# mkofler96/DeepSDF

Hardware: AMD Instinct MI355X
Metric: SDF point-samples/sec per training step (8x512 decoder, 16384 pts) (higher is better)
Workload: dtype f32; 1 GPU; configs[1]: 64 synthetic sphere-SDF scenes, latent_dim=256, 8x512 decoder + layer-4 skip, weight-norm, dropout 0.2, 16384 pts/step (64 scenes x 256 samples), fp32; headline_config=True, parallelism=dp1

## Files before the change

deepsdf_amd/csrc/dsdf_api.hip:

```cpp
#include "../../include/dsdf.h"

#include <hip/hip_runtime.h>
#include <math.h>
#include <stdarg.h>
#include <stdio.h>
#include <string.h>

#include <stdlib.h>

#include <algorithm>
#include <atomic>

#include "dwstream.hpp"
#include "sample.hpp"
#include "fused.hpp"
#include "fused_bf16x8.hpp"
#include "gemm.hpp"
#include "kernels.hpp"
#include "mcubes.hpp"
#include "meshsdf.hpp"
#include "msgrid.hpp"

using namespace dsdf;

// ... 240 lines not shown
}

std::atomic<size_t> g_redzone{0};
struct WsRow { const char* name; int idx; size_t off, bytes; };
struct WsTable {
  int n, dropped;
  size_t total;
  WsRow row[DSDF_WS_MAX_REGIONS];
  void reset() { n = 0; dropped = 0; total = 0; }
  void add(const char* name, int idx, size_t off, size_t bytes) {
    if (n < DSDF_WS_MAX_REGIONS) row[n++] = WsRow{name, idx, off, bytes};
    else ++dropped;
  }
};
thread_local WsTable t_last_plan;

struct Plan {
  int nl, W0, N, R;
  int ld_in[DSDF_MAX_LAYERS];
  size_t in_off[DSDF_MAX_LAYERS];
  int ld_dp, ldz, ldcs, ld_part, last_blocks, nsplit, kchunk, mt;
  long long slab;
  size_t u_off, y_off, dp_off[2], dzA_off, dzB_off, slab_off, colsum_off, part_off, part2_off, partdb_off,
      partloss_off, segpart_off, segnorm_off, gnorm_off, dxz_off[2], lnpg_off, lnpb_off, total;
  size_t lnx_off[DSDF_MAX_LAYERS], lnr_off[DSDF_MAX_LAYERS];
  size_t dpl_off[DSDF_MAX_LAYERS], mask_off[DSDF_MAX_LAYERS], cs_off[DSDF_MAX_LAYERS], dwslab_off[DSDF_MAX_LAYERS];
  int nwg, frows;
  DwSched dw;
  DwSched dwph[DSDF_MAX_BUCKETS];
  int dw_nb, dw_cut[DSDF_MAX_BUCKETS + 1];
  int segmode, ldu, ldh;
  long long hstride;
  size_t hoistU_off, xsum_off[2], hs_off, zr_off;
};

Plan make_plan(const DsdfNet* n, int64_t N, int64_t R, bool inference, bool segmode = false, int nb = 2, int frows = FROWS,
               WsTable* rec = nullptr) {
  Plan P;
  memset(&P, 0, sizeof(P));
  P.frows = frows;
  P.nl = n->n_layers; P.W0 = n->latent_size + n->geom_dim; P.N = (int)N; P.R = (int)R;
  size_t o = 0;
  const size_t guard = g_redzone.load(std::memory_order_relaxed);
  if (rec) rec->reset();
  auto take = [&](const char* name, int idx, size_t bytes) {
    size_t r = o;
    o += (size_t)rup((int64_t)bytes, 256) + guard;
    if (rec) rec->add(name, idx, r, bytes);
    return r;
  };
  int maxw = 4;
  for (int l = 0; l < P.nl; ++l) {
    P.ld_in[l] = (int)rup(n->in_dim[l], 4);
    if (P.ld_in[l] > maxw) maxw = P.ld_in[l];
  }
  if (inference) {
// ... 33 lines not shown
  int maxout = 1;
  for (int l = 0; l < P.nl - 1; ++l) {
    const int64_t s = (int64_t)n->out_dim[l] * P.ld_in[l];
    if (s > maxslab) maxslab = s;
    if (n->out_dim[l] > maxout) maxout = n->out_dim[l];
  }
  P.slab = rup(maxslab, 64);
  P.slab_off = take("slab", -1, (size_t)P.nsplit * P.slab * 4);
  P.mt = (int)((N + BM - 1) / BM);
  P.ldcs = (int)rup(maxout, 4);
  P.colsum_off = take("colsum", -1, (size_t)P.mt * P.ldcs * 4);
  if (n->ln_param_mask) { P.lnpg_off = take("lnpg", -1, (size_t)LN_BLOCKS * P.ldcs * 4); P.lnpb_off = take("lnpb", -1, (size_t)LN_BLOCKS * P.ldcs * 4); }
  P.last_blocks = (int)((N + 15) / 16);
  if (P.last_blocks > LAST_BLOCKS_MAX) P.last_blocks = LAST_BLOCKS_MAX;
  if (P.last_blocks < 1) P.last_blocks = 1;
  P.ld_part = 2 * P.ld_in[P.nl - 1];
  const size_t part_rows = (size_t)std::max<int64_t>(P.last_blocks, (N + frows - 1) / frows);
  P.part_off = take("part", -1, part_rows * P.ld_part * 4);
  P.part2_off = take("part2", -1, (size_t)LAST_GROUPS * P.ld_part * 4);
  P.partdb_off = take("partdb", -1, part_rows * 4);
  P.partloss_off = take("partloss", -1, part_rows * 4);
  P.segpart_off = take("segpart", -1, (size_t)LAT_SLICES_MAX * (R > 0 ? R : 1) * (n->latent_size > 0 ? n->latent_size : 1) * 4);
  P.segnorm_off = take("segnorm", -1, (size_t)(R > 0 ? R : 1) * 4);
  P.gnorm_off = take("gnorm", -1, 1024 * 4);
  P.nwg = (int)((N + frows - 1) / frows);
  for (int l = 0; l < P.nl - 1; ++l) {
    P.dpl_off[l] = take("dpl", l, (size_t)N * maxw * 4 + 4096);
    P.mask_off[l] = take("mask", l, (size_t)P.nwg * 256 * 16);
    P.cs_off[l] = take("cs", l, (size_t)P.nwg * P.ldcs * 4);
  }
  P.dw = dw_schedule(n, N, P.ld_in, segmode);
  P.dw_nb = nb < 2 ? 2 : (nb > DSDF_MAX_BUCKETS ? DSDF_MAX_BUCKETS : nb);
  dw_bucket_cuts(n, P.dw_nb, P.dw_cut);
  for (int t = 0; t < P.dw_nb; ++t)
    P.dwph[t] = dw_schedule(n, N, P.ld_in, segmode, P.dw_cut[t + 1], P.dw_cut[t],
                            t == 0 && P.dw_nb == 2 && segmode && P.nwg <= chip_waves() / 4 ? 64 : 0);
  for (int l = 0; l < P.nl - 1; ++l) {
    int ns = P.dw.nsplit[l];
    for (int t = 0; t < P.dw_nb; ++t)
      if (P.dwph[t].nsplit[l] > ns) ns = P.dwph[t].nsplit[l];
    P.dwslab_off[l] = take("dwslab", l, (size_t)ns * P.dw.slab[l] * 4);
  }
  P.segmode = segmode ? 1 : 0;
  if (segmode) {
    P.ldu = P.ldcs;
    P.hoistU_off = take("hoistU", -1, (size_t)(R > 0 ? R : 1) * 2 * P.ldu * 4);
    for (int t = 0; t < 2; ++t) P.xsum_off[t] = take("xsum", t, (size_t)P.nwg * 4 * P.ldcs * 4);
// ... 41 lines not shown
int launch_last(const LastArgs& a, int blocks, hipStream_t st) {
  if (a.n <= 0) return 0;
  const int in = a.in;
  ProfScope ps(DSDF_PROF_LAST, (MODE == LAST_FWD ? 2.0 : 6.0) * a.n * a.in, st);
  if (in <= 256) hipLaunchKernelGGL((last_layer_kernel<MODE, 1>), dim3(blocks), dim3(256), 0, st, a);
  else if (in <= 512) hipLaunchKernelGGL((last_layer_kernel<MODE, 2>), dim3(blocks), dim3(256), 0, st, a);
  else if (in <= 1024) hipLaunchKernelGGL((last_layer_kernel<MODE, 4>), dim3(blocks), dim3(256), 0, st, a);
  else hipLaunchKernelGGL((last_layer_kernel<MODE, 8>), dim3(blocks), dim3(256), 0, st, a);
  LAUNCH_OK("last_layer_kernel");
  return 0;
}

AdamRide adam_ride(float* p, const float* g, float* m, float* v, int64_t n, float lr, const DsdfAdamCfg* c) {
  AdamRide a;
  memset(&a, 0, sizeof(a));
  const double bc1 = 1.0 - pow((double)c->beta1, (double)c->step), bc2 = 1.0 - pow((double)c->beta2, (double)c->step);
  a.p = p; a.g = g; a.m = m; a.v = v; a.n = n;
  a.blocks = (int)((n + 255) / 256 < 2048 ? (n + 255) / 256 : 2048);
  a.omb1 = 1.0f - c->beta1; a.b2 = c->beta2; a.omb2 = 1.0f - c->beta2;
  a.step_size = (float)((double)lr / bc1); a.bc2_sqrt = (float)sqrt(bc2); a.eps = c->eps;
  return a;
}

int materialize(const DsdfNet* net, const float* params, float* packed, hipStream_t st, bool scales_ready = false,
                const AdamRide* ride = nullptr) {
  DsdfParamLayout L;
  param_layout(net, &L);
  const Packed pk = packed_layout(net);
  WnAll a;
  memset(&a, 0, sizeof(a));
  a.nl = net->n_layers;
  a.scale = packed + pk.scale_off;
  int rows = 0, tiles = 0;
  for (int l = 0; l < net->n_layers; ++l) {
    WnLayer& y = a.ly[l];
    y.v = params + L.v_off[l];
    y.g = L.g_off[l] >= 0 ? params + L.g_off[l] : nullptr;
    y.W = packed + pk.w_off[l];
    y.WT = (l == net->n_layers - 1) ? nullptr : packed + pk.wt_off[l];
    y.out = net->out_dim[l]; y.in = net->in_dim[l]; y.ldw = pk.ldw[l]; y.ldwt = pk.ldwt[l];
    y.row0 = rows; y.tile0 = tiles; y.tcols = (y.in + 31) / 32;
    const bool last = l == net->n_layers - 1;
    y.Wf = last ? nullptr : packed + pk.wf_off[l];
    y.WTf = last ? nullptr : packed + pk.wtf_off[l];
    y.Wfb = (last || !net->fwd_bf16) ? nullptr : reinterpret_cast<__bf16*>(packed + pk.wfb_off[l]);
    y.Uf = pk.uf[l]; y.UTf = pk.utf[l];
    const bool sp = net->gemm_split && !last;
    y.Ws = sp ? reinterpret_cast<__bf16*>(packed + pk.ws_off[l]) : nullptr;
    y.WTs = sp ? reinterpret_cast<__bf16*>(packed + pk.wts_off[l]) : nullptr;
    y.ws_plane = pk.ws_plane[l]; y.wts_plane = pk.wts_plane[l];
    rows += y.out;
    tiles += ((y.out + 31) / 32) * y.tcols;
  }
  a.total_rows = rows; a.total_tiles = tiles;
  if (!scales_ready) {
    hipLaunchKernelGGL(wn_scale_kernel, dim3((rows + 3) / 4), dim3(256), 0, st, a);
    LAUNCH_OK("wn_scale_kernel");
  }
  if (ride != nullptr) a.adam = *ride;
  hipLaunchKernelGGL(wn_tiles_kernel, dim3(tiles + a.adam.blocks), dim3(256), 0, st, a);
  LAUNCH_OK("wn_tiles_kernel");
  return 0;
}

constexpr float LATENT_DROPOUT_P = 0.2f;
constexpr int LATENT_DROPOUT_KEY = DSDF_MAX_LAYERS - 1;
inline uint32_t latent_drop_thr() { return (uint32_t)lround((double)LATENT_DROPOUT_P * 65536.0); }
inline bool net_variant(const DsdfNet* n) { return n->latent_dropout || n->xyz_in_all || n->ln_param_mask != 0; }
inline bool ln_applied(const DsdfNet* n, int l) { return ((n->ln_param_mask >> l) & 1) && l < n->n_layers - 1; }


int run_gather(const DsdfNet* net, const Plan& P, void* ws, const float* table, const DsdfBatch* b, const float* input,
               int64_t ld_in, int64_t n, hipStream_t st, int training = 0, const uint32_t* keys = nullptr, uint32_t row_offset = 0) {
  GatherArgs g;
  memset(&g, 0, sizeof(g));
  g.table = table; g.L = net->latent_size; g.G = net->geom_dim;
  if (b) { g.xyz = b->xyz; g.seg_scene = b->seg_scene; g.seg_offset = b->seg_offset; g.R = (int)b->n_segments; }
// ... 57 lines not shown
int run_hoist(const DsdfNet* net, const Plan& P, void* ws, const float* packed, const float* table, const DsdfBatch* b,
              FusedSeg* seg, hipStream_t st, const HoistRenorm* renorm = nullptr) {
  if (net->latent_size < 1 || net->latent_size > HOIST_MAXL)
    return fail(DSDF_E_INVALID, "segment mode needs 1 <= latent_size <= %d (got %d)", HOIST_MAXL, net->latent_size);
  const Packed pk = packed_layout(net);
  const int ks = skip_layer(net);
  HoistArgs h;
  memset(&h, 0, sizeof(h));
  memset(seg, 0, sizeof(*seg));
  h.nh = ks > 0 ? 2 : 1;
  h.W[0] = packed + pk.w_off[0]; h.ldw[0] = pk.ldw[0]; h.c0[0] = 0; h.out[0] = net->out_dim[0];
  seg->h[0].layer = 0; seg->h[0].wx = h.W[0] + net->latent_size; seg->h[0].ldw = pk.ldw[0];
  seg->h[1].layer = -1;
  if (ks > 0) {
    h.W[1] = packed + pk.w_off[ks]; h.ldw[1] = pk.ldw[ks]; h.c0[1] = net->out_dim[ks - 1]; h.out[1] = net->out_dim[ks];
    seg->h[1].layer = ks; seg->h[1].wx = h.W[1] + h.c0[1] + net->latent_size; seg->h[1].ldw = pk.ldw[ks];
  }
  h.L = net->latent_size; h.seg_scene = b->seg_scene; h.table = table; h.R = (int)b->n_segments;
  h.U = at<float>(ws, P.hoistU_off); h.ldu = P.ldu;
  h.bf16 = net->fwd_bf16 ? 1 : 0;
  if (renorm != nullptr) {
    h.max_norm = renorm->max_norm; h.zr = at<float>(ws, P.zr_off);
    h.dlat = renorm->nzero > 0 ? renorm->dlat : nullptr; h.nzero = renorm->nzero;
  }
  const int rows = h.out[0] + (ks > 0 ? h.out[1] : 0);
  const dim3 hgrid((unsigned)((rows + 3) / 4), (unsigned)((h.R + HOIST_SC - 1) / HOIST_SC));
  switch ((h.L + 63) >> 6) {
    case 1: hipLaunchKernelGGL(seg_hoist_kernel<1>, hgrid, dim3(256), 0, st, h); break;
    case 2: hipLaunchKernelGGL(seg_hoist_kernel<2>, hgrid, dim3(256), 0, st, h); break;
    case 3: case 4: hipLaunchKernelGGL(seg_hoist_kernel<4>, hgrid, dim3(256), 0, st, h); break;
    default: hipLaunchKernelGGL(seg_hoist_kernel<8>, hgrid, dim3(256), 0, st, h); break;
  }
  LAUNCH_OK("seg_hoist_kernel");
  seg->wg_per_seg = (int)(b->seg_len / P.frows);
  seg->xyz = b->xyz; seg->G = net->geom_dim; seg->U = h.U; seg->ldu = h.ldu;
  return 0;
}

int run_fused_forward(const DsdfNet* net, const Plan& P, void* ws, const float* packed, const float* params, int64_t n,
                      int training, const uint32_t* keys, uint32_t row_offset, bool store_act, float* y_out, float* u_out,
                      hipStream_t st, const FusedSeg* seg = nullptr, FusedFwdArgs* defer = nullptr) {
  DsdfParamLayout L;
  param_layout(net, &L);
  const Packed pk = packed_layout(net);
  const int last = net->n_layers - 1;
  FusedFwdArgs a;
// ... 214 lines not shown
      TRY(launch_nt<EPI_BWD>(a, st));
      if (want_xyz) {
        const long long tot = (long long)n * net->geom_dim;
        hipLaunchKernelGGL(acc_cols_kernel, dim3((unsigned)((tot + 255) / 256)), dim3(256), 0, st, at<float>(ws, P.dxz_off[0]), 4,
                           at<float>(ws, P.dxz_off[1]), 4, 0, (int)n, net->geom_dim, *xyz_acc ? 1 : 0);
        LAUNCH_OK("acc_cols_kernel");
        *xyz_acc = true;
      }
      cur ^= 1;
    } else if (ncols_dz > 0) {
      a.C = at<float>(ws, P.dzA_off); a.ldc = P.ldz; a.N = ncols_dz;
      TRY(launch_nt<EPI_PLAIN>(a, st));
      if (net->latent_dropout && training && keys != nullptr && net->latent_size > 0) {
        const long long tot = (long long)n * net->latent_size;
        hipLaunchKernelGGL(latent_drop_bwd_kernel, dim3((unsigned)((tot + 255) / 256)), dim3(256), 0, st, at<float>(ws, P.dzA_off), P.ldz,
                           (int)n, net->latent_size, keys[LATENT_DROPOUT_KEY], latent_drop_thr(), 1.0f / (1.0f - LATENT_DROPOUT_P), row_offset);
        LAUNCH_OK("latent_drop_bwd_kernel");
      }
    }
  }
  return 0;
}

struct FuseAdam { const DsdfAdamCfg* cfg; float* params; float* exp_avg; float* exp_avg_sq; float* packed; };

struct SegBwd { const FusedSeg* seg; const int64_t* seg_scene; const float* table; int R;
                ScatterArgs* scatter; bool* scatter_done;
                const float* zr; };

int run_backward_fused(const DsdfNet* net, const Plan& P, void* ws, const float* packed, const float* params, int64_t n,
                       int training, float* grads, int accumulate, int ncols_dz, bool* used_dzB, hipStream_t st,
                       bool want_dw, const FusedBwdHead& head, const FuseAdam* fz = nullptr, const SegBwd* sb = nullptr,
                       const FusedFwdArgs* fwd = nullptr,
                       int phase = 0) {
  const DwSched& DS = phase == 0 ? P.dw : P.dwph[phase - 1];
  auto in_phase = [&](int l) { return phase == 0 || (l >= P.dw_cut[phase] && l < P.dw_cut[phase - 1]); };
  DsdfParamLayout L;
  param_layout(net, &L);
  const Packed pk = packed_layout(net);
  const int nl = net->n_layers, last = nl - 1;
  *used_dzB = false;
  FusedBwdArgs a;
  memset(&a, 0, sizeof(a));
  a.N = (int)n;
  a.head = head;
  const bool segmode = sb != nullptr;
  const int ks = skip_layer(net);
// ... 192 lines not shown
      if (segmode && (l == 0 || l == ks)) {
        f.hoist = 1; f.lat0 = l == 0 ? 0 : net->out_dim[l - 1]; f.hW = net->latent_size + net->geom_dim; f.ldh = P.ldh;
        f.hs = at<float>(ws, P.hs_off) + (l == 0 ? 0 : P.hstride);
      }
      if (fz != nullptr) {
        const DsdfAdamCfg* c = fz->cfg;
        const double bc1 = 1.0 - pow((double)c->beta1, (double)c->step), bc2 = 1.0 - pow((double)c->beta2, (double)c->step);
        f.adam = 1;
        f.pb = fz->params + L.bias_off[l]; f.mb = fz->exp_avg + L.bias_off[l]; f.sb = fz->exp_avg_sq + L.bias_off[l];
        f.pv = fz->params + L.v_off[l];    f.mv = fz->exp_avg + L.v_off[l];    f.sv = fz->exp_avg_sq + L.v_off[l];
        if (L.g_off[l] >= 0) { f.pg = fz->params + L.g_off[l]; f.mg = fz->exp_avg + L.g_off[l]; f.sg = fz->exp_avg_sq + L.g_off[l]; }
        int r0 = 0;
        for (int q = 0; q < l; ++q) r0 += net->out_dim[q];
        f.scale_out = fz->packed + pk.scale_off + r0;
        f.omb1 = 1.0f - c->beta1; f.b2 = c->beta2; f.omb2 = 1.0f - c->beta2;
        f.step_size = (float)((double)c->lr_decoder / bc1); f.bc2_sqrt = (float)sqrt(bc2); f.eps = c->eps;
      }
      fa.row0[fa.n] = rows;
      rows += fin_blocks(f.out, f.in);
      ++fa.n;
    }
    fa.row0[fa.n] = rows;
    if (rows == 0) return 0;
    if (segmode && sb->scatter != nullptr && phase <= 1) {
      hipLaunchKernelGGL(finalize_scatter_kernel, dim3(rows + sb->R), dim3(256), 0, st, fa, *sb->scatter, rows);
      LAUNCH_OK("finalize_scatter_kernel");
      *sb->scatter_done = true;
    } else {
      hipLaunchKernelGGL(finalize_all_kernel, dim3(rows), dim3(256), 0, st, fa);
      LAUNCH_OK("finalize_all_kernel");
    }
  }
  return 0;
}

FusedBwdHead make_head(const DsdfNet* net, const Plan& P, void* ws, const float* packed, const float* params, int mode,
                       int training) {
  DsdfParamLayout L;
  param_layout(net, &L);
  const Packed pk = packed_layout(net);
  const int last = net->n_layers - 1;
  FusedBwdHead h;
  memset(&h, 0, sizeof(h));
  h.mode = mode;
  h.a_last = at<float>(ws, P.in_off[last]); h.ld_a = P.ld_in[last]; h.in_last = net->in_dim[last];
  h.w_last = packed + pk.w_off[last]; h.b_last = params + L.bias_off[last]; h.use_tanh = net->use_tanh;
  h.mask_scale = mask_scale_of(net, last - 1, training);
// ... 600 lines not shown
    }
    a.total_rows = rows;
    hipLaunchKernelGGL(adam_rows_kernel, dim3((rows + 3) / 4), dim3(256), 0, st, a);
    LAUNCH_OK("adam_rows_kernel");
    for (int l = 0; l < net->n_layers; ++l)
      if (L.ln_w_off[l] >= 0)
        TRY(adam_launch(params + L.ln_w_off[l], grads + L.ln_w_off[l], exp_avg + L.ln_w_off[l], exp_avg_sq + L.ln_w_off[l],
                        2 * (int64_t)net->out_dim[l], cfg->lr_decoder, cfg, cfg->grad_scale, st));
  }
  if (n_latent_floats > 0) {
    if (!latent_table || !dlat || !lat_exp_avg || !lat_exp_avg_sq) return fail(DSDF_E_INVALID, "NULL latent argument");
    const AdamRide ride = adam_ride(latent_table, dlat, lat_exp_avg, lat_exp_avg_sq, n_latent_floats, cfg->lr_latent, cfg);
    return materialize(net, params, packed, st, true, &ride);
  }
  return materialize(net, params, packed, st, true);
}

int dsdf_train_step(const DsdfNet* net, float* packed, float* params, float* grads, float* exp_avg, float* exp_avg_sq,
                    float* latent_table, int64_t n_scenes, float* dlat, float* lat_exp_avg, float* lat_exp_avg_sq,
                    const DsdfBatch* b, const DsdfLossCfg* cfg, const DsdfAdamCfg* adam, float* loss_out, float* sdf_out,
                    void* ws, size_t ws_bytes, void* stream) {
  if (!adam || !exp_avg || !exp_avg_sq || !lat_exp_avg || !lat_exp_avg_sq) return fail(DSDF_E_INVALID, "NULL argument");
  if (adam->step < 1) return fail(DSDF_E_INVALID, "Adam step must be >= 1");
  FuseAdam fz{adam, params, exp_avg, exp_avg_sq, packed};
  int fused = 0;
  const bool can_fuse = adam->grad_scale == nullptr && cfg && !cfg->frozen_decoder;
  TRY(train_fb_impl(net, packed, params, latent_table, n_scenes, b, cfg, grads, dlat, loss_out, sdf_out, 0, ws, ws_bytes, stream,
                    can_fuse ? &fz : nullptr, &fused));
  const int64_t nlat = n_scenes * net->latent_size;
  if (!fused)
    return dsdf_adam_step(net, params, grads, exp_avg, exp_avg_sq, latent_table, dlat, lat_exp_avg, lat_exp_avg_sq, nlat, adam,
                          packed, stream);
  hipStream_t st = (hipStream_t)stream;
  const AdamRide ride = adam_ride(latent_table, dlat, lat_exp_avg, lat_exp_avg_sq, nlat, adam->lr_latent, adam);
  return materialize(net, params, packed, st, true, &ride);
}

int dsdf_adam_latent_only(float* latent, const float* dlat, float* exp_avg, float* exp_avg_sq, int64_t n,
                          const DsdfAdamCfg* cfg, void* stream) {
  if (!latent || !dlat || !exp_avg || !exp_avg_sq || !cfg || n <= 0) return fail(DSDF_E_INVALID, "bad arguments");
  if (cfg->step < 1) return fail(DSDF_E_INVALID, "Adam step must be >= 1");
  return adam_launch(latent, dlat, exp_avg, exp_avg_sq, n, cfg->lr_latent, cfg, nullptr, (hipStream_t)stream);
}

int dsdf_adam_latent_sched(float* latent, const float* dlat, float* exp_avg, float* exp_avg_sq, int64_t n, const float* sched,
                           int64_t n_steps, int64_t* step_counter, float beta1, float beta2, float eps, float l2_coef, void* stream) {
  if (!latent || !dlat || !exp_avg || !exp_avg_sq || !sched || !step_counter || n <= 0 || n_steps <= 0)
    return fail(DSDF_E_INVALID, "bad arguments");
  hipStream_t st = (hipStream_t)stream;
  int blocks = (int)((n + 255) / 256);
  if (blocks > 2048) blocks = 2048;
  hipLaunchKernelGGL(adam_sched_kernel, dim3(blocks), dim3(256), 0, st, latent, dlat, exp_avg, exp_avg_sq, (long long)n, sched,
                     (long long)n_steps, (const long long*)step_counter, 1.0f - beta1, beta2, 1.0f - beta2, eps, l2_coef);
  LAUNCH_OK("adam_sched_kernel");
  hipLaunchKernelGGL(counter_inc_kernel, dim3(1), dim3(1), 0, st, (long long*)step_counter);
  LAUNCH_OK("counter_inc_kernel");
  return 0;
// ... 413 lines not shown
```

deepsdf_amd/csrc/kernels.hpp:

```cpp
#pragma once
#include "common.hpp"

namespace dsdf {

constexpr int FSEG_MAXW = 512;

__global__ void latent_renorm_kernel(float* __restrict__ table, int L, const int64_t* __restrict__ seg_scene,
                                     int R, float max_norm, float* __restrict__ dlat, long long nzero) {
  if (dlat != nullptr)
    for (long long i = ((long long)blockIdx.x * blockDim.x + threadIdx.x) * 4; i < nzero; i += (long long)gridDim.x * blockDim.x * 4) {
      if (i + 3 < nzero) *reinterpret_cast<float4*>(dlat + i) = make_float4(0.f, 0.f, 0.f, 0.f);
      else for (long long q = i; q < nzero; ++q) dlat[q] = 0.f;
    }
  const int r = blockIdx.x * (blockDim.x >> 6) + (threadIdx.x >> 6);
  const int lane = threadIdx.x & 63;
  if (r >= R || max_norm <= 0.f) return;
  const int64_t j = seg_scene[r];
  int dup = 0;
  for (int q = lane; q < r; q += 64) dup |= (seg_scene[q] == j);
  if (__any(dup)) return;
  float* row = table + (size_t)j * L;
  float ss = 0.f;
  for (int c = lane; c < L; c += 64) { const float v = row[c]; ss += v * v; }
  ss = wave_sum(ss);
// ... 65 lines not shown
  if (i >= (long long)n * G) return;
  const int r = (int)(i / G), j = (int)(i % G);
  const float u = u_in[r];
  const float t1 = use_tanh ? tanhf(u) : u;
  const float y = tanhf(t1);
  float du = d_sdf[r] * (1.f - y * y);
  if (use_tanh) du *= (1.f - t1 * t1);
  float* q = dst + (size_t)r * ldd + c0 + j;
  const float v = du * w_xyz[j];
  *q = accumulate ? *q + v : v;
}

constexpr int HOIST_MAXL = 512;
constexpr int HOIST_SC = 16;
struct HoistArgs {
  int nh;
  const float* W[2]; int ldw[2]; int c0[2]; int out[2];
  int L; const int64_t* seg_scene; const float* table; int R;
  float* U; int ldu;
  int bf16;
  float max_norm;
  float* zr;
  float* dlat; long long nzero;
};
template <int KU>
__device__ __forceinline__ void seg_hoist_body(const HoistArgs& p, const int n, const int t) {
  const int lane = threadIdx.x & 63;
  const int s0 = blockIdx.y * HOIST_SC;
  const long long myscene = (long long)p.seg_scene[min(s0 + (lane & (HOIST_SC - 1)), p.R - 1)];
  const float* wrow = p.W[t] + (size_t)n * p.ldw[t] + p.c0[t];
  float wv[KU], v[HOIST_SC][KU];
#pragma unroll
  for (int k = 0; k < KU; ++k) wv[k] = wrow[min(lane + 64 * k, p.L - 1)];
#pragma unroll
  for (int q = 0; q < HOIST_SC; ++q) {
    const float* row = p.table + (size_t)__shfl(myscene, q, 64) * p.L;
#pragma unroll
    for (int k = 0; k < KU; ++k) v[q][k] = row[min(lane + 64 * k, p.L - 1)];
  }
#pragma unroll
  for (int k = 0; k < KU; ++k) {
    const bool ok = lane + 64 * k < p.L;
    wv[k] = ok ? wv[k] : 0.f;
#pragma unroll
    for (int q = 0; q < HOIST_SC; ++q) v[q][k] = ok ? v[q][k] : 0.f;
  }
// ... 30 lines not shown
  for (int q = 0; q < HOIST_SC; ++q) a[q] = 0.f;
#pragma unroll
  for (int k = 0; k < KU; ++k) {
    const float w = p.bf16 ? (float)(__bf16)wv[k] : wv[k];
#pragma unroll
    for (int q = 0; q < HOIST_SC; ++q) {
      const float x = p.bf16 ? (float)(__bf16)v[q][k] : v[q][k];
      if (lane + 64 * k < p.L) a[q] = fmaf(w, x, a[q]);
    }
  }
  const float r = wave_sum16(a, lane);
  const int qi = wave_sum16_index(lane);
  if ((lane & 3) == 0 && s0 + qi < p.R) p.U[((size_t)(s0 + qi) * 2 + t) * p.ldu + n] = r;
}
template <int KU>
__global__ __launch_bounds__(256) void seg_hoist_kernel(const HoistArgs p) {
  if (p.dlat != nullptr) {
    const long long nb = (long long)gridDim.x * gridDim.y, b = (long long)blockIdx.y * gridDim.x + blockIdx.x;
    for (long long i = (b * 256 + threadIdx.x) * 4; i < p.nzero; i += nb * 256 * 4) {
      if (i + 3 < p.nzero) *reinterpret_cast<float4*>(p.dlat + i) = make_float4(0.f, 0.f, 0.f, 0.f);
      else for (long long q = i; q < p.nzero; ++q) p.dlat[q] = 0.f;
    }
  }
  int n = blockIdx.x * 4 + (threadIdx.x >> 6);
  int t = 0;
  if (n >= p.out[0]) { n -= p.out[0]; t = 1; }
  if (t >= p.nh || n >= p.out[t]) return;
  seg_hoist_body<KU>(p, n, t);
}

constexpr int SDW_ROWS_RIDE = 32, SDW_ROWS_WIDE = 8;
constexpr int SDW_LDS_FLOATS = 64 * SDW_ROWS_RIDE + 256 * 4 + 2 * 64;
struct SegDwArgs {
  int nh; const float* cs[2]; const float* xsum[2]; int out[2];
  int ldcs, nwg, wg_per_seg, R, L, G;
  const int64_t* seg_scene; const float* table;
  const float* zr;
  float* HS; int ldh; long long hstride;
};
template <int SDW_ROWS>
__device__ __forceinline__ void seg_dw_body(const SegDwArgs& p, int bidx, float* lds) {
  constexpr int SDW_SLOTS = 256 / SDW_ROWS;
  float (*css)[SDW_ROWS] = reinterpret_cast<float (*)[SDW_ROWS]>(lds);
  float (*xred)[SDW_ROWS][4] = reinterpret_cast<float (*)[SDW_ROWS][4]>(lds + 64 * SDW_ROWS);
  long long* srow = reinterpret_cast<long long*>(lds + 64 * SDW_ROWS + SDW_SLOTS * SDW_ROWS * 4);
  const int tid = threadIdx.x;
// ... 135 lines not shown
  float* p; const float* g; float* m; float* v; long long n; int blocks;
  float omb1, b2, omb2, step_size, bc2_sqrt, eps;
};
struct WnAll { int nl; int total_rows; int total_tiles; float* scale; AdamRide adam; WnLayer ly[DSDF_MAX_LAYERS]; };

__global__ __launch_bounds__(256) void wn_scale_kernel(const WnAll p) {
  const int gr = blockIdx.x * 4 + (threadIdx.x >> 6), lane = threadIdx.x & 63;
  if (gr >= p.total_rows) return;
  int l = 0;
  while (l + 1 < p.nl && gr >= p.ly[l + 1].row0) ++l;
  const WnLayer& L = p.ly[l];
  const int row = gr - L.row0;
  float s = 1.f;
  if (L.g != nullptr) {
    const float* vr = L.v + (size_t)row * L.in;
    float ss = 0.f;
    for (int c = lane; c < L.in; c += 64) { const float x = vr[c]; ss += x * x; }
    ss = wave_sum(ss);
    s = L.g[row] / sqrtf(ss);
  }
  if (lane == 0) p.scale[gr] = s;
}

__global__ __launch_bounds__(256) void wn_tiles_kernel(const WnAll p) {
  __shared__ float tile[32][33];
  const int t = blockIdx.x;
  if (t >= p.total_tiles) {
    const AdamRide& a = p.adam;
    for (long long i = (long long)(t - p.total_tiles) * 256 + threadIdx.x; i < a.n; i += (long long)a.blocks * 256) {
      const float gi = a.g[i];
      const float mi = fmaf(a.omb1, gi - a.m[i], a.m[i]);
      const float vi = a.b2 * a.v[i] + a.omb2 * gi * gi;
      a.m[i] = mi; a.v[i] = vi;
      a.p[i] = a.p[i] - a.step_size * (mi / (sqrtf(vi) / a.bc2_sqrt + a.eps));
    }
    return;
  }
  int l = 0;
  while (l + 1 < p.nl && t >= p.ly[l + 1].tile0) ++l;
  const WnLayer& L = p.ly[l];
  const int tt = t - L.tile0;
  const int rb = tt / L.tcols, cb = tt % L.tcols;
  const int r0 = rb * 32, c0 = cb * 32;
  const int tx = threadIdx.x & 31, ty = threadIdx.x >> 5;
#pragma unroll
  for (int k = 0; k < 4; ++k) {
    const int rr = ty + 8 * k, row = r0 + rr, col = c0 + tx;
    float w = 0.f;
    if (row < L.out && col < L.in) {
      w = L.v[(size_t)row * L.in + col] * p.scale[L.row0 + row];
      L.W[(size_t)row * L.ldw + col] = w;
    }
    tile[rr][tx] = w;
  }
  if (L.WT == nullptr && L.Wf == nullptr && L.Wfb == nullptr && L.Ws == nullptr) return;
  __syncthreads();
  if (L.WT != nullptr) {
#pragma unroll
    for (int k = 0; k < 4; ++k) {
      const int cc = ty + 8 * k, col = c0 + cc, row = r0 + tx;
      if (col < L.in && row < L.out) L.WT[(size_t)col * L.ldwt + row] = tile[tx][cc];
    }
  }
  const int uu = threadIdx.x >> 7, i = (threadIdx.x >> 6) & 1, lane = threadIdx.x & 63;
  const int fr = lane & 31, fh = lane >> 5, kk = 16 * uu + 8 * fh + 4 * i;
  if (L.Wf != nullptr) {
    float4 v4 = make_float4(tile[fr][kk], tile[fr][kk + 1], tile[fr][kk + 2], tile[fr][kk + 3]);
    *reinterpret_cast<float4*>(L.Wf + ((size_t)(rb * L.Uf + 2 * cb + uu) * 2 + i) * 256 + lane * 4) = v4;
  }
  if (L.Wfb != nullptr) {
    typedef __bf16 bf16x4 __attribute__((ext_vector_type(4)));
    const bf16x4 h4 = {(__bf16)tile[fr][kk], (__bf16)tile[fr][kk + 1], (__bf16)tile[fr][kk + 2], (__bf16)tile[fr][kk + 3]};
    const int slot = (cb & 1) * 16 + 2 * (cb >> 1) + uu;
    *reinterpret_cast<bf16x4*>(L.Wfb + ((size_t)(rb * 32 + slot) * 64 + lane) * 8 + 4 * i) = h4;
  }
  if (L.WTf != nullptr) {
    float4 v4 = make_float4(tile[kk][fr], tile[kk + 1][fr], tile[kk + 2][fr], tile[kk + 3][fr]);
    *reinterpret_cast<float4*>(L.WTf + ((size_t)(cb * L.UTf + 2 * rb + uu) * 2 + i) * 256 + lane * 4) = v4;
  }
// ... 737 lines not shown
    }
    seg_dw_body<RIDE ? SDW_ROWS_RIDE : SDW_ROWS_WIDE>(p.dw, i, lds);
    return;
  }
  i -= p.dw_n;
  if constexpr (RIDE) seg_latgrad_all_body(p.lat, i, lat_n, lds);
  else seg_latgrad_body(p.lat, i % p.lat_bx, i / p.lat_bx, lds);
}
__device__ __attribute__((noinline)) void post_bwd_role_ride(const PostBwdArgs& p, int i, int lat_n, float* lds) {
  post_bwd_role<true>(p, i, lat_n, lds);
}
__global__ __launch_bounds__(256) void post_bwd_kernel(const PostBwdArgs p, const int lat_n) {
  __shared__ __attribute__((aligned(16))) float lds[ROLE_LDS_FLOATS];
  post_bwd_role<false>(p, blockIdx.x, lat_n, lds);
}

struct ScatterArgs {
  const float* segpart; const float* segnorm; const int64_t* seg_scene; const int64_t* seg_offset; int R; int L;
  float* table; float* dlat; float creg;
  int nslice; long long slice_stride;
  const float* zr;
  const float* part_loss; int n_part; float loss_scale; float* loss_out; int accumulate;
};
__device__ __forceinline__ void seg_scatter_body(const ScatterArgs& p, int r) {
  __shared__ float red[4];
  __shared__ int dup;
  const int tid = threadIdx.x;
  if (r == 0) {
    float s = 0.f;
    if (p.creg != 0.f)
      for (int q = tid; q < p.R; q += 256) s += p.creg * (float)(p.seg_offset[q + 1] - p.seg_offset[q]) * p.segnorm[q];
    s = block_sum_256(s, red);
    float d = 0.f;
    for (int q = tid; q < p.n_part; q += 256) d += p.part_loss[q];
    d = block_sum_256(d, red);
    if (tid == 0) {
      const float v = d * p.loss_scale + s;
      *p.loss_out = p.accumulate ? *p.loss_out + v : v;
    }
  }
  const int64_t j = p.seg_scene[r];
  if (tid == 0) dup = 0;
  __syncthreads();
  int d = 0;
  for (int q = tid; q < r; q += 256) d |= (p.seg_scene[q] == j);
  if (d) dup = 1;
  __syncthreads();
  if (dup) return;
  for (int c = tid; c < p.L; c += 256) {
    const float z = p.zr != nullptr ? p.zr[(size_t)r * p.L + c] : p.table[(size_t)j * p.L + c];
    float acc = 0.f;
    for (int q = r; q < p.R; ++q) {
      if (q != r && p.seg_scene[q] != j) continue;
      float v = p.segpart[(size_t)q * p.L + c];
      for (int sl = 1; sl < p.nslice; ++sl) v += p.segpart[(size_t)sl * p.slice_stride + (size_t)q * p.L + c];
      if (p.creg != 0.f) {
        const float nrm = p.segnorm[q];
        if (nrm > 0.f) v += p.creg * (float)(p.seg_offset[q + 1] - p.seg_offset[q]) * z / nrm;
      }
      acc += v;
    }
    p.dlat[(size_t)j * p.L + c] += acc;
    if (p.zr != nullptr) p.table[(size_t)j * p.L + c] = z;
  }
}

__global__ __launch_bounds__(256) void seg_scatter_kernel(const ScatterArgs p) { seg_scatter_body(p, blockIdx.x); }

__global__ __launch_bounds__(256) void finalize_scatter_kernel(const FinAll p, const ScatterArgs sc, const int rows) {
  if ((int)blockIdx.x < sc.R) { seg_scatter_body(sc, (int)blockIdx.x); return; }
  __shared__ float red[4];
  finalize_block(p, (int)blockIdx.x - sc.R, red);
}

__global__ __launch_bounds__(256) void adam_kernel(float* __restrict__ p, const float* __restrict__ g,
                                                   float* __restrict__ m, float* __restrict__ v, long long n,
                                                   float one_minus_b1, float b2, float one_minus_b2, float step_size,
                                                   float bc2_sqrt, float eps, const float* gscale) {
  const float gs = gscale ? *gscale : 1.f;
  for (long long i = (long long)blockIdx.x * 256 + threadIdx.x; i < n; i += (long long)gridDim.x * 256) {
    const float gi = g[i] * gs;
    const float mi = fmaf(one_minus_b1, gi - m[i], m[i]);
    const float vi = b2 * v[i] + one_minus_b2 * gi * gi;
    m[i] = mi; v[i] = vi;
    p[i] = p[i] - step_size * (mi / (sqrtf(vi) / bc2_sqrt + eps));
  }
}

__global__ __launch_bounds__(256) void adam_sched_kernel(float* __restrict__ p, const float* __restrict__ g, float* __restrict__ m,
                                                         float* __restrict__ v, long long n, const float* __restrict__ sched,
                                                         long long n_steps, const long long* __restrict__ counter, float one_minus_b1,
                                                         float b2, float one_minus_b2, float eps, float l2) {
  long long it = *counter;
  if (it >= n_steps) it = n_steps - 1;
  const float step_size = sched[2 * it], bc2_sqrt = sched[2 * it + 1];
// ... 191 lines not shown
```

Baseline: 13.09 million point-samples/s.

## Fuse weight-norm materialization and latent Adam into finalize-scatter tail kernel

Adds a finalize_tail_kernel that, in segmented training with fused Adam, runs the per-row finalize (decoder Adam plus weight-norm scale), the latent scatter with an inline latent Adam update, the Adam update for latent rows outside the batch, and the weight-norm re-materialization of each 32-row block. The last finishing block of each group is chosen with atomic counters. This removes the separate materialize/wn_tiles launch and one extra pass over the latent table after the backward pass. In exchange it adds atomic counters reset in the hoist kernel, acquire/release fences, and a per-latent-row duplicate scan over the batch scenes, and it can be turned off with DSDF_NO_TAIL.

```diff
diff --git a/deepsdf_amd/csrc/dsdf_api.hip b/deepsdf_amd/csrc/dsdf_api.hip
--- a/deepsdf_amd/csrc/dsdf_api.hip
+++ b/deepsdf_amd/csrc/dsdf_api.hip
@@ -286,7 +286,7 @@
   int ld_dp, ldz, ldcs, ld_part, last_blocks, nsplit, kchunk, mt;
   long long slab;
   size_t u_off, y_off, dp_off[2], dzA_off, dzB_off, slab_off, colsum_off, part_off, part2_off, partdb_off,
-      partloss_off, segpart_off, segnorm_off, gnorm_off, dxz_off[2], lnpg_off, lnpb_off, total;
+      partloss_off, segpart_off, segnorm_off, dxz_off[2], lnpg_off, lnpb_off, total;
   size_t lnx_off[DSDF_MAX_LAYERS], lnr_off[DSDF_MAX_LAYERS];
   size_t dpl_off[DSDF_MAX_LAYERS], mask_off[DSDF_MAX_LAYERS], cs_off[DSDF_MAX_LAYERS], dwslab_off[DSDF_MAX_LAYERS];
   int nwg, frows;
@@ -296,6 +296,7 @@
   int segmode, ldu, ldh;
   long long hstride;
   size_t hoistU_off, xsum_off[2], hs_off, zr_off;
+  size_t tailcnt_off; int tail_groups;
 };
 
 Plan make_plan(const DsdfNet* n, int64_t N, int64_t R, bool inference, bool segmode = false, int nb = 2, int frows = FROWS,
@@ -375,7 +376,9 @@
   P.partloss_off = take("partloss", -1, part_rows * 4);
   P.segpart_off = take("segpart", -1, (size_t)LAT_SLICES_MAX * (R > 0 ? R : 1) * (n->latent_size > 0 ? n->latent_size : 1) * 4);
   P.segnorm_off = take("segnorm", -1, (size_t)(R > 0 ? R : 1) * 4);
-  P.gnorm_off = take("gnorm", -1, 1024 * 4);
+  for (int l = 0; l < P.nl; ++l) P.tail_groups += (n->out_dim[l] + TAIL_ROWS - 1) / TAIL_ROWS;
+  if (P.tail_groups > TAIL_MAXGROUPS) P.tail_groups = 0;
+  P.tailcnt_off = take("tailcnt", -1, (size_t)TAIL_MAXGROUPS * 4);
   P.nwg = (int)((N + frows - 1) / frows);
   for (int l = 0; l < P.nl - 1; ++l) {
     P.dpl_off[l] = take("dpl", l, (size_t)N * maxw * 4 + 4096);
@@ -463,8 +466,7 @@
   return a;
 }
 
-int materialize(const DsdfNet* net, const float* params, float* packed, hipStream_t st, bool scales_ready = false,
-                const AdamRide* ride = nullptr) {
+WnAll wn_all(const DsdfNet* net, const float* params, float* packed) {
   DsdfParamLayout L;
   param_layout(net, &L);
   const Packed pk = packed_layout(net);
@@ -494,6 +496,12 @@
     tiles += ((y.out + 31) / 32) * y.tcols;
   }
   a.total_rows = rows; a.total_tiles = tiles;
+  return a;
+}
+int materialize(const DsdfNet* net, const float* params, float* packed, hipStream_t st, bool scales_ready = false,
+                const AdamRide* ride = nullptr) {
+  WnAll a = wn_all(net, params, packed);
+  const int rows = a.total_rows, tiles = a.total_tiles;
   if (!scales_ready) {
     hipLaunchKernelGGL(wn_scale_kernel, dim3((rows + 3) / 4), dim3(256), 0, st, a);
     LAUNCH_OK("wn_scale_kernel");
@@ -597,6 +605,7 @@
   if (renorm != nullptr) {
     h.max_norm = renorm->max_norm; h.zr = at<float>(ws, P.zr_off);
     h.dlat = renorm->nzero > 0 ? renorm->dlat : nullptr; h.nzero = renorm->nzero;
+    h.cnt = at<int>(ws, P.tailcnt_off); h.ncnt = TAIL_MAXGROUPS;
   }
   const int rows = h.out[0] + (ks > 0 ? h.out[1] : 0);
   const dim3 hgrid((unsigned)((rows + 3) / 4), (unsigned)((h.R + HOIST_SC - 1) / HOIST_SC));
@@ -857,7 +866,8 @@
   return 0;
 }
 
-struct FuseAdam { const DsdfAdamCfg* cfg; float* params; float* exp_avg; float* exp_avg_sq; float* packed; };
+struct FuseAdam { const DsdfAdamCfg* cfg; float* params; float* exp_avg; float* exp_avg_sq; float* packed;
+                  const AdamRide* ride; bool* tail_done; };
 
 struct SegBwd { const FusedSeg* seg; const int64_t* seg_scene; const float* table; int R;
                 ScatterArgs* scatter; bool* scatter_done;
@@ -1096,7 +1106,27 @@
     }
     fa.row0[fa.n] = rows;
     if (rows == 0) return 0;
-    if (segmode && sb->scatter != nullptr && phase <= 1) {
+    static const bool no_tail = [] { const char* e = getenv("DSDF_NO_TAIL"); return e && e[0] == '1'; }();
+    bool tail = segmode && sb->scatter != nullptr && phase == 0 && fz != nullptr && fz->ride != nullptr && !no_tail &&
+                sb->scatter->table == fz->ride->p && sb->scatter->dlat == fz->ride->g &&
+                fz->ride->n % net->latent_size == 0 && fa.n == net->n_layers && P.tail_groups > 0;
+    for (int l = 0; l < net->n_layers; ++l) tail = tail && net->in_dim[l] <= 32 * TAIL_MAXT && net->in_dim[l] <= 64 * FW_MAXK;
+    if (tail) {
+      WnAll wa = wn_all(net, fz->params, fz->packed);
+      wa.adam = *fz->ride;
+      TailArgs tl;
+      memset(&tl, 0, sizeof(tl));
+      tl.cnt = at<int>(ws, P.tailcnt_off);
+      tl.adam_rows = wa.adam.n / net->latent_size;
+      wa.adam.blocks = (int)std::min<long long>(std::max<long long>(tl.adam_rows, 1), 2048);
+      int g0[DSDF_MAX_LAYERS], g = 0;
+      for (int l = 0; l < net->n_layers; ++l) { g0[l] = g; g += (net->out_dim[l] + TAIL_ROWS - 1) / TAIL_ROWS; }
+      for (int k = 0; k < fa.n; ++k) { tl.layer[k] = last - k; tl.grp0[k] = g0[last - k]; }
+      hipLaunchKernelGGL(finalize_tail_kernel, dim3(rows + sb->R + wa.adam.blocks), dim3(256), 0, st, fa, *sb->scatter, wa, tl, rows);
+      LAUNCH_OK("finalize_tail_kernel");
+      *sb->scatter_done = true;
+      *fz->tail_done = true;
+    } else if (segmode && sb->scatter != nullptr && phase <= 1) {
       hipLaunchKernelGGL(finalize_scatter_kernel, dim3(rows + sb->R), dim3(256), 0, st, fa, *sb->scatter, rows);
       LAUNCH_OK("finalize_scatter_kernel");
       *sb->scatter_done = true;
@@ -1743,17 +1773,20 @@
                     void* ws, size_t ws_bytes, void* stream) {
   if (!adam || !exp_avg || !exp_avg_sq || !lat_exp_avg || !lat_exp_avg_sq) return fail(DSDF_E_INVALID, "NULL argument");
   if (adam->step < 1) return fail(DSDF_E_INVALID, "Adam step must be >= 1");
-  FuseAdam fz{adam, params, exp_avg, exp_avg_sq, packed};
+  if (!net) return fail(DSDF_E_INVALID, "NULL argument");
+  const int64_t nlat = n_scenes * net->latent_size;
+  const AdamRide ride = adam_ride(latent_table, dlat, lat_exp_avg, lat_exp_avg_sq, nlat, adam->lr_latent, adam);
+  bool tail_done = false;
+  FuseAdam fz{adam, params, exp_avg, exp_avg_sq, packed, nlat > 0 ? &ride : nullptr, &tail_done};
   int fused = 0;
   const bool can_fuse = adam->grad_scale == nullptr && cfg && !cfg->frozen_decoder;
   TRY(train_fb_impl(net, packed, params, latent_table, n_scenes, b, cfg, grads, dlat, loss_out, sdf_out, 0, ws, ws_bytes, stream,
                     can_fuse ? &fz : nullptr, &fused));
-  const int64_t nlat = n_scenes * net->latent_size;
   if (!fused)
     return dsdf_adam_step(net, params, grads, exp_avg, exp_avg_sq, latent_table, dlat, lat_exp_avg, lat_exp_avg_sq, nlat, adam,
                           packed, stream);
+  if (tail_done) return 0;
   hipStream_t st = (hipStream_t)stream;
-  const AdamRide ride = adam_ride(latent_table, dlat, lat_exp_avg, lat_exp_avg_sq, nlat, adam->lr_latent, adam);
   return materialize(net, params, packed, st, true, &ride);
 }
 
diff --git a/deepsdf_amd/csrc/kernels.hpp b/deepsdf_amd/csrc/kernels.hpp
--- a/deepsdf_amd/csrc/kernels.hpp
+++ b/deepsdf_amd/csrc/kernels.hpp
@@ -111,6 +111,7 @@
   float max_norm;
   float* zr;
   float* dlat; long long nzero;
+  int* cnt; int ncnt;
 };
 template <int KU>
 __device__ __forceinline__ void seg_hoist_body(const HoistArgs& p, const int n, const int t) {
@@ -187,6 +188,8 @@
       else for (long long q = i; q < p.nzero; ++q) p.dlat[q] = 0.f;
     }
   }
+  if (p.cnt != nullptr && blockIdx.x == 0 && blockIdx.y == 0)
+    for (int i = threadIdx.x; i < p.ncnt; i += 256) p.cnt[i] = 0;
   int n = blockIdx.x * 4 + (threadIdx.x >> 6);
   int t = 0;
   if (n >= p.out[0]) { n -= p.out[0]; t = 1; }
@@ -368,18 +371,20 @@
   if (lane == 0) p.scale[gr] = s;
 }
 
+__device__ __forceinline__ void adam_ride_elem(const AdamRide& a, const long long i, const float gi, const float pi) {
+  const float mi = fmaf(a.omb1, gi - a.m[i], a.m[i]);
+  const float vi = fmaf(gi, a.omb2 * gi, a.b2 * a.v[i]);
+  a.m[i] = mi; a.v[i] = vi;
+  a.p[i] = fmaf(-a.step_size, mi / (sqrtf(vi) / a.bc2_sqrt + a.eps), pi);
+}
+__device__ __forceinline__ void wn_tile_out(const WnLayer& L, const int rb, const int cb, const float (&tile)[32][33]);
 __global__ __launch_bounds__(256) void wn_tiles_kernel(const WnAll p) {
   __shared__ float tile[32][33];
   const int t = blockIdx.x;
   if (t >= p.total_tiles) {
     const AdamRide& a = p.adam;
-    for (long long i = (long long)(t - p.total_tiles) * 256 + threadIdx.x; i < a.n; i += (long long)a.blocks * 256) {
-      const float gi = a.g[i];
-      const float mi = fmaf(a.omb1, gi - a.m[i], a.m[i]);
-      const float vi = a.b2 * a.v[i] + a.omb2 * gi * gi;
-      a.m[i] = mi; a.v[i] = vi;
-      a.p[i] = a.p[i] - a.step_size * (mi / (sqrtf(vi) / a.bc2_sqrt + a.eps));
-    }
+    for (long long i = (long long)(t - p.total_tiles) * 256 + threadIdx.x; i < a.n; i += (long long)a.blocks * 256)
+      adam_ride_elem(a, i, a.g[i], a.p[i]);
     return;
   }
   int l = 0;
@@ -401,6 +406,11 @@
   }
   if (L.WT == nullptr && L.Wf == nullptr && L.Wfb == nullptr && L.Ws == nullptr) return;
   __syncthreads();
+  wn_tile_out(L, rb, cb, tile);
+}
+__device__ __forceinline__ void wn_tile_out(const WnLayer& L, const int rb, const int cb, const float (&tile)[32][33]) {
+  const int r0 = rb * 32, c0 = cb * 32;
+  const int tx = threadIdx.x & 31, ty = threadIdx.x >> 5;
   if (L.WT != nullptr) {
 #pragma unroll
     for (int k = 0; k < 4; ++k) {
@@ -1184,7 +1194,7 @@
   const float* zr;
   const float* part_loss; int n_part; float loss_scale; float* loss_out; int accumulate;
 };
-__device__ __forceinline__ void seg_scatter_body(const ScatterArgs& p, int r) {
+__device__ __forceinline__ void seg_scatter_body(const ScatterArgs& p, int r, const AdamRide* ad = nullptr) {
   __shared__ float red[4];
   __shared__ int dup;
   const int tid = threadIdx.x;
@@ -1222,8 +1232,10 @@
       }
       acc += v;
     }
-    p.dlat[(size_t)j * p.L + c] += acc;
-    if (p.zr != nullptr) p.table[(size_t)j * p.L + c] = z;
+    const float gsum = p.dlat[(size_t)j * p.L + c] + acc;
+    p.dlat[(size_t)j * p.L + c] = gsum;
+    if (ad != nullptr) adam_ride_elem(*ad, (long long)j * p.L + c, gsum, z);
+    else if (p.zr != nullptr) p.table[(size_t)j * p.L + c] = z;
   }
 }
 
@@ -1233,6 +1245,95 @@
   if ((int)blockIdx.x < sc.R) { seg_scatter_body(sc, (int)blockIdx.x); return; }
   __shared__ float red[4];
   finalize_block(p, (int)blockIdx.x - sc.R, red);
+}
+
+struct TailArgs {
+  int* cnt;
+  int grp0[DSDF_MAX_LAYERS];
+  int layer[DSDF_MAX_LAYERS];
+  long long adam_rows;
+};
+constexpr int TAIL_ROWS = 32;
+constexpr int TAIL_MAXT = 16;
+constexpr int TAIL_MAXGROUPS = 1024;
+__device__ __forceinline__ void wn_rowblock(const WnLayer& L, const float* scale, const int rb, float (&tile)[32][33]) {
+  const int tx = threadIdx.x & 31, ty = threadIdx.x >> 5, r0 = rb * 32;
+  float w[TAIL_MAXT][4], s[4];
+#pragma unroll
+  for (int k = 0; k < 4; ++k) s[k] = scale[L.row0 + min(r0 + ty + 8 * k, L.out - 1)];
+#pragma unroll
+  for (int cb = 0; cb < TAIL_MAXT; ++cb)
+#pragma unroll
+    for (int k = 0; k < 4; ++k)
+      w[cb][k] = L.v[(size_t)min(r0 + ty + 8 * k, L.out - 1) * L.in + min(cb * 32 + tx, L.in - 1)];
+  const bool copies = L.WT != nullptr || L.Wf != nullptr || L.Wfb != nullptr || L.Ws != nullptr;
+#pragma unroll
+  for (int cb = 0; cb < TAIL_MAXT; ++cb) {
+    if (cb >= L.tcols) break;
+#pragma unroll
+    for (int k = 0; k < 4; ++k) {
+      const int rr = ty + 8 * k, row = r0 + rr, col = cb * 32 + tx;
+      float x = 0.f;
+      if (row < L.out && col < L.in) {
+        x = w[cb][k] * s[k];
+        L.W[(size_t)row * L.ldw + col] = x;
+      }
+      tile[rr][tx] = x;
+    }
+    if (copies) {
+      __syncthreads();
+      wn_tile_out(L, rb, cb, tile);
+      __syncthreads();
+    }
+  }
+}
+__global__ __launch_bounds__(256) void finalize_tail_kernel(const FinAll p, const ScatterArgs sc, const WnAll wn, const TailArgs tl,
+                                                            const int rows) {
+  __shared__ float tile[32][33];
+  __shared__ int flag;
+  int b = (int)blockIdx.x;
+  const AdamRide* ad = wn.adam.blocks > 0 ? &wn.adam : nullptr;
+  if (b < sc.R) { seg_scatter_body(sc, b, ad); return; }
+  b -= sc.R;
+  if (b >= rows) {
+    for (long long j = b - rows; j < tl.adam_rows; j += wn.adam.blocks) {
+      if (threadIdx.x == 0) flag = 0;
+      __syncthreads();
+      int d = 0;
+      for (int q = threadIdx.x; q < sc.R; q += 256) d |= (sc.seg_scene[q] == j);
+      if (d) flag = 1;
+      __syncthreads();
+      const bool in_batch = flag != 0;
+      __syncthreads();
+      if (in_batch) continue;
+      for (int c = threadIdx.x; c < sc.L; c += 256) {
+        const long long i = j * sc.L + c;
+        adam_ride_elem(wn.adam, i, wn.adam.g[i], wn.adam.p[i]);
+      }
+    }
+    return;
+  }
+  finalize_block(p, b, &tile[0][0]);
+  int k = 0;
+  while (k + 1 < p.n && b >= p.row0[k + 1]) ++k;
+  const int lb = b - p.row0[k], nb = p.row0[k + 1] - p.row0[k];
+  const int grp = lb / (TAIL_ROWS / 4), need = min(TAIL_ROWS / 4, nb - grp * (TAIL_ROWS / 4));
+  int* cnt = tl.cnt + tl.grp0[k] + grp;
+  asm volatile("s_waitcnt vmcnt(0)" ::: "memory");
+  __syncthreads();
+  if (threadIdx.x == 0) {
+    __builtin_amdgcn_fence(__ATOMIC_RELEASE, "agent");
+    asm volatile("s_waitcnt vmcnt(0)" ::: "memory");
+    const int last = __hip_atomic_fetch_add(cnt, 1, __ATOMIC_RELAXED, __HIP_MEMORY_SCOPE_AGENT) == need - 1;
+    if (last) {
+      __hip_atomic_store(cnt, 0, __ATOMIC_RELAXED, __HIP_MEMORY_SCOPE_AGENT);
+      __builtin_amdgcn_fence(__ATOMIC_ACQUIRE, "agent");
+      asm volatile("s_waitcnt vmcnt(0)" ::: "memory");
+    }
+    flag = last;
+  }
+  __syncthreads();
+  if (flag) wn_rowblock(wn.ly[tl.layer[k]], wn.scale, grp, tile);
 }
 
 __global__ __launch_bounds__(256) void adam_kernel(float* __restrict__ p, const float* __restrict__ g,
```

Result: slower. 10.81 million point-samples/s (-17.4%).
